# liuyuan-pal/Gen6D

Measured on NVIDIA H100. Metric: poses/sec end-to-end (128^2 crop, 64 refs, 3 refine iters), higher is better.
Workload: dtype f32

## Files before the change

### gen6d_b200/csrc/conv_tc.cu

```cuda
#include <cuda_fp16.h>
#include <string.h>

#include "tc_common.cuh"

namespace g6d {

constexpr int TC_BM = 128;
constexpr int TC_PRODUCER_WARPS = 8;
constexpr int TC_CONSUMER_WARPS = 8;
constexpr int TC_THREADS = (TC_PRODUCER_WARPS + TC_CONSUMER_WARPS) * 32;
constexpr int TC_ISSUER = TC_PRODUCER_WARPS * 32;
constexpr int TC_PRODUCER_REGS = 96, TC_CONSUMER_REGS = 160;
static_assert(TC_PRODUCER_WARPS * TC_PRODUCER_REGS + TC_CONSUMER_WARPS * TC_CONSUMER_REGS <= 65536 / 32, "register file of one SM");
constexpr int TC_FOLD_PRODUCER_REGS = 40, TC_FOLD_CONSUMER_REGS = 216;
static_assert(TC_PRODUCER_WARPS * TC_FOLD_PRODUCER_REGS + TC_CONSUMER_WARPS * TC_FOLD_CONSUMER_REGS <= 65536 / 32, "register file of one SM");
static_assert(TC_BM == 64 * (TC_CONSUMER_WARPS / 4), "one 64-row wgmma tile per consumer warpgroup");
constexpr int TC_MAX_K_PER_CHAIN = 2048;

template <int KIND> struct KindCfg;
template <> struct KindCfg<G6D_TC_TF32> {
    static constexpr int BK = 32;
    static constexpr int NV = 1;
    static constexpr float CROSS = 1.f;
};
template <> struct KindCfg<G6D_TC_F16> {
    static constexpr int BK = 64;
    static constexpr int NV = 2;
    static constexpr float CROSS = 1.f / 2048.f;
};
constexpr float F16_LO_SCALE = 2048.f;
constexpr int TC2_RING = 2, FLAT_RING = 3;
__host__ __device__ __forceinline__ int f16_k_source(int p) {
    const int c = p >> 3, i = p & 7;
    return i < 4 ? 4 * c + i : 32 + 4 * c + (i - 4);
}

struct ConvTcP {
    const float* x; const float* bias; const float* ps; const float* pb;
    float* y; float* ws;
    int B, D, H, W, Cin, ics, ico, Cout, kd, kh, kw, stride, pd, ph, pw, Do, Ho, Wo, ocs, oco, pro, act;
    long long group_rows;
    int M, K, kblocks, splits, kb_per_split;
    double* stats; long long stats_rows;
    int split_in;
    int reuse_order;
    int fold;
};

__device__ __forceinline__ void kblock_src(const ConvTcP& p, int sp, int it, int& tap, int& cb) {
    if (p.reuse_order) {
        const int taps2 = p.kh * p.kw;
        const int u = it / taps2, t = it - u * taps2;
        cb = sp * (p.kb_per_split / (taps2 * p.kd)) + u / p.kd;
        tap = (u % p.kd) * taps2 + t;
    } else {
        const int cblocks = p.Cin / 64, kb = sp * p.kb_per_split + it;
        tap = kb / cblocks;
        cb = kb - tap * cblocks;
    }
}

struct KbIter {
    int kx, ky, kz, cb;
    __device__ __forceinline__ void start(const ConvTcP& p, int sp, int it) {
        int tap;
        kblock_src(p, sp, it, tap, cb);
        kx = tap % p.kw;
        const int tq = tap / p.kw;
        ky = tq % p.kh;
        kz = tq / p.kh;
    }
    __device__ __forceinline__ void next(const ConvTcP& p) {
        if (p.reuse_order) {
            if (++kx < p.kw) return;
            kx = 0;
            if (++ky < p.kh) return;
            ky = 0;
            if (++kz < p.kd) return;
            kz = 0; ++cb;
// ... 167 lines not shown
    for (int i = 0; i < BN / 8; ++i) {
#pragma unroll
        for (int e = 0; e < 2; ++e) {
            const float y0 = dst0 ? cross[4 * i + e] : 0.f, y1 = dst1 ? cross[4 * i + 2 + e] : 0.f;
            const float2 s = slice_moments(y0, y1);
            const int n = n_base + 8 * i + cq + e;
            if (lane < 4 && n < Cout) {
                atomicAdd(stats + (group * Cout + n) * 2, (double)s.x);
                atomicAdd(stats + (group * Cout + n) * 2 + 1, (double)s.y);
            }
        }
    }
}

template <int BN, int KIND>
__device__ __forceinline__ void epilogue_tile(float (&acc)[AccCfg<BN>::NMAIN][BN / 2], float (&cross)[BN / 2], int n_acc,
                                              float* dst0, float* dst1, int n_base, int Cout, const float* __restrict__ bias,
                                              int act, bool partial, bool vec2, double* __restrict__ stats, long long group,
                                              int lane) {
    sum_chains<BN, KIND>(acc, cross, n_acc);
    store_tile<BN>(cross, dst0, dst1, n_base, Cout, bias, act, partial, vec2, stats, group, lane);
}

constexpr int TC2_PF_BYTES = 12 * 128;

template <int BN> struct Tc2Cfg {
    static constexpr int A_BYTES = TC_BM * 128;
    static constexpr int B_BYTES = BN * 128;
    static constexpr int STAGE_BYTES = 2 * A_BYTES + 2 * B_BYTES;
    static constexpr int STAGES = (208 * 1024) / STAGE_BYTES > 6 ? 6 : (208 * 1024) / STAGE_BYTES;
    static constexpr int SMEM_BYTES = STAGES * STAGE_BYTES + 1024 + 256;
};

struct Tc2Work { int m_tiles, n_tiles, total; };

template <int BN, int KIND, bool FOLD>
__global__ void __launch_bounds__(TC_THREADS, 1)
conv_tc2_kernel(const ConvTcP p, const Tc2Work wk, const __grid_constant__ CUtensorMap map_hi,
                const __grid_constant__ CUtensorMap map_lo, const __grid_constant__ CUtensorMap map_a) {
    using Cfg = Tc2Cfg<BN>;
    using KC = KindCfg<KIND>;
    constexpr int NPW = TC_PRODUCER_WARPS;
    constexpr int STAGES = Cfg::STAGES;
    constexpr int NMAIN = AccCfg<BN>::NMAIN;
    constexpr int BK = KC::BK, NV = KC::NV;
    constexpr int RSTEP = NPW * 4;
    constexpr int ROWS = TC_BM / RSTEP;
    constexpr int RING = TC2_RING;
    constexpr int PF = TC2_PF_BYTES / 128;
    extern __shared__ uint8_t smem_raw[];
    const uint32_t base = (smem_u32(smem_raw) + 1023u) & ~1023u;
    const uint32_t bar_base = base + STAGES * Cfg::STAGE_BYTES;
    auto a_hi = [&](int s) { return base + s * Cfg::STAGE_BYTES; };
    auto a_lo = [&](int s) { return base + s * Cfg::STAGE_BYTES + Cfg::A_BYTES; };
    auto b_hi = [&](int s) { return base + s * Cfg::STAGE_BYTES + 2 * Cfg::A_BYTES; };
    auto b_lo = [&](int s) { return base + s * Cfg::STAGE_BYTES + 2 * Cfg::A_BYTES + Cfg::B_BYTES; };
    auto full_a = [&](int s) { return bar_base + 8 * s; };
    auto full_b = [&](int s) { return bar_base + 8 * (STAGES + s); };
    auto empty = [&](int s) { return bar_base + 8 * (2 * STAGES + s); };

    const int warp = threadIdx.x >> 5, lane = threadIdx.x & 31;
    if (threadIdx.x == TC_ISSUER) {
        for (int s = 0; s < STAGES; ++s) {
            mbar_init(full_a(s), p.split_in ? 1 : NPW);
            mbar_init(full_b(s), 1);
            mbar_init(empty(s), TC_CONSUMER_WARPS);
        }
        fence_barrier_init();
        asm volatile("prefetch.tensormap [%0];" ::"l"(&map_hi) : "memory");
        asm volatile("prefetch.tensormap [%0];" ::"l"(&map_lo) : "memory");
        if (p.split_in) asm volatile("prefetch.tensormap [%0];" ::"l"(&map_a) : "memory");
    }
    __syncthreads();

    auto decode = [&](int w, int& mt, int& nt, int& sp) {
        nt = w % wk.n_tiles; w /= wk.n_tiles;
        mt = w % wk.m_tiles;
        sp = w / wk.m_tiles;
    };
    auto kblocks_of = [&](int sp) { return min(p.kblocks, sp * p.kb_per_split + p.kb_per_split) - sp * p.kb_per_split; };
    const int chains = FOLD ? p.splits : 1;
    auto chain_of = [&](int j, int& mt, int& nt, int& sp) {
        const int w = blockIdx.x + (j / chains) * gridDim.x;
        if (w >= wk.total) return false;
        decode(w, mt, nt, sp);
        sp += j % chains;
        return true;
    };

    if (warp < NPW) {
        setmaxnreg_dec<FOLD ? TC_FOLD_PRODUCER_REGS : TC_PRODUCER_REGS>();
        if (FOLD || p.split_in) {
            if (threadIdx.x == 0) {
                const bool vol = p.D > 1 || p.kd > 1;
                int g = 0;
                int mt, nt, sp;
                for (int j = 0; chain_of(j, mt, nt, sp); ++j) {
                    const int nkb = kblocks_of(sp);
                    int m = mt * TC_BM;
                    const int xo = m % p.Wo; m /= p.Wo;
                    const int yo = m % p.Ho; m /= p.Ho;
                    const int zo = m % p.Do;
                    const int b = m / p.Do;
                    KbIter pf, k;
                    pf.start(p, sp, 0);
                    k = pf;
                    auto prefetch = [&]() {
                        const int kc = pf.tap(p) * p.Cin + pf.cb * BK;
                        tma_prefetch_2d(&map_hi, kc, nt * BN);
                        tma_prefetch_2d(&map_lo, kc, nt * BN);
                        pf.next(p);
                    };
#pragma unroll 1
                    for (int i = 0; i < min(nkb, PF - 1); ++i) prefetch();
                    for (int it = 0; it < nkb; ++it, ++g, k.next(p)) {
                        if (it + PF - 1 < nkb) prefetch();
                        const int tap = k.tap(p), cb = k.cb;
                        const uint16_t ox = (uint16_t)k.kx, oy = (uint16_t)k.ky, oz = (uint16_t)k.kz;
                        const int s = g % STAGES;
                        mbar_wait(empty(s), ((g / STAGES) & 1) ^ 1, 1, g);
                        mbar_expect_tx(full_b(s), 2 * Cfg::B_BYTES);
                        tma_load_2d(b_hi(s), &map_hi, full_b(s), tap * p.Cin + cb * BK, nt * BN);
                        tma_load_2d(b_lo(s), &map_lo, full_b(s), tap * p.Cin + cb * BK, nt * BN);
                        mbar_expect_tx(full_a(s), 2 * Cfg::A_BYTES);
                        if (vol) {
                            tma_im2col_5d(a_hi(s), &map_a, full_a(s), 2 * BK * cb, xo - p.pw, yo - p.ph, zo - p.pd, b, ox, oy, oz);
// ... 75 lines not shown
                }
                if (e == 0) mbar_wait(empty(s), (n_use & 1) ^ 1, 1, g_it);
#pragma unroll
                for (int j = 0; j < ROWS; ++j) {
                    const int r = r0 + RSTEP * j;
                    const uint32_t so = r * 128 + ((chunk ^ (r & 7)) << 4);
                    split_store<KIND>(a_hi(s) + so, a_lo(s) + so, v[q][j], e);
                }
                if (e == NV - 1) {
                    fence_proxy_async();
                    __syncwarp();
                    if (lane == 0) mbar_arrive(full_a(s));
                }
            };
            const int ncol = nkb * NV;
#pragma unroll
            for (int q = 0; q < RING - 1; ++q)
                if (q < ncol) issue_loads(q, q % NV);
            for (int u = 0; u < ncol; u += RING) {
#pragma unroll
                for (int q = 0; q < RING; ++q) {
                    if (u + q < ncol) {
                        if (u + q + RING - 1 < ncol) issue_loads((q + RING - 1) % RING, (u + q + RING - 1) % NV);
                        process(q, (u + q) % NV, (u + q) / NV);
                    }
                }
            }
            git += nkb;
        }
    } else {
        setmaxnreg_inc<FOLD ? TC_FOLD_CONSUMER_REGS : TC_CONSUMER_REGS>();
        const int cw = warp - NPW;
        const uint32_t a_row = (cw >> 2) * 64 * 128;
        const bool issuer = !FOLD && threadIdx.x == TC_ISSUER && !p.split_in;
        int lw = blockIdx.x, lit = 0, lg = 0;
        auto load_next = [&]() {
            int mt, nt, sp, nkb = 0;
            for (; lw < wk.total; lw += gridDim.x, lit = 0) {
                decode(lw, mt, nt, sp);
                nkb = kblocks_of(sp);
                if (lit < nkb) break;
            }
            if (lw >= wk.total) return;
            const int kb_begin = sp * p.kb_per_split;
            if (lit == 0) {
                for (int i = 0; i < min(nkb, PF); ++i) {
                    tma_prefetch_2d(&map_hi, (kb_begin + i) * BK, nt * BN);
                    tma_prefetch_2d(&map_lo, (kb_begin + i) * BK, nt * BN);
                }
            } else if (lit + PF - 1 < nkb) {
                tma_prefetch_2d(&map_hi, (kb_begin + lit + PF - 1) * BK, nt * BN);
                tma_prefetch_2d(&map_lo, (kb_begin + lit + PF - 1) * BK, nt * BN);
            }
            const int s = lg % STAGES;
            mbar_wait(empty(s), ((lg / STAGES) & 1) ^ 1, 3, lg);
            mbar_expect_tx(full_b(s), 2 * Cfg::B_BYTES);
            tma_load_2d(b_hi(s), &map_hi, full_b(s), (kb_begin + lit) * BK, nt * BN);
            tma_load_2d(b_lo(s), &map_lo, full_b(s), (kb_begin + lit) * BK, nt * BN);
            ++lit; ++lg;
        };
        auto release = [&](int g) {
            __syncwarp();
            if (lane == 0) mbar_arrive(empty(g % STAGES));
            if (issuer) load_next();
        };
        if (issuer)
            for (int i = 0; i < STAGES; ++i) load_next();

        float acc[NMAIN][BN / 2];
        float cross[BN / 2];
        float run[FOLD ? BN / 2 : 1];
        int g = 0;
        int mt, nt, sp;
        for (int j = 0; chain_of(j, mt, nt, sp); ++j) {
            const int nkb = kblocks_of(sp);
            zero_acc<BN, NMAIN>(acc, cross);
            for (int it0 = 0; it0 < nkb; it0 += NMAIN) {
#pragma unroll
                for (int a = 0; a < NMAIN; ++a) {
                    const int it = it0 + a;
                    if (it < nkb) {
                        const int s = g % STAGES;
                        mbar_wait(full_a(s), (g / STAGES) & 1, 4, g);
                        mbar_wait(full_b(s), (g / STAGES) & 1, 5, g);
                        mma_stage<BN, KIND>(acc[a], cross, a_hi(s) + a_row, a_lo(s) + a_row, b_hi(s), b_lo(s));
                        wgmma_wait<1>();
                        if (it > 0) release(g - 1);
                        ++g;
                    }
                }
            }
            wgmma_wait<0>();
            if (nkb > 0) release(g - 1);

            sum_chains<BN, KIND>(acc, cross, nkb < NMAIN ? nkb : NMAIN);
            if constexpr (FOLD) {
#pragma unroll
                for (int jj = 0; jj < BN / 2; ++jj) run[jj] = (sp == 0 ? 0.f : run[jj]) + cross[jj];
                if (sp < p.splits - 1) continue;
#pragma unroll
                for (int jj = 0; jj < BN / 2; ++jj) cross[jj] = run[jj];
            }
            const bool partial = p.splits > 1 && !FOLD;
            const int n_base = nt * BN;
            const int m0 = mt * TC_BM + 16 * cw + (lane >> 2), m1 = m0 + 8;
            float* out = partial ? p.ws + (long long)sp * p.M * p.Cout + n_base : p.y + p.oco + n_base;
            const long long ld = partial ? p.Cout : p.ocs;
            const bool vec2 = partial ? (p.Cout & 1) == 0
                                      : ((p.ocs & 1) == 0 && (p.oco & 1) == 0 && (reinterpret_cast<uintptr_t>(p.y) & 7) == 0);
            store_tile<BN>(cross, m0 < p.M ? out + m0 * ld : nullptr, m1 < p.M ? out + m1 * ld : nullptr, n_base, p.Cout, p.bias,
                           p.act, partial, vec2, p.stats, (long long)(mt * TC_BM + 16 * cw) / p.stats_rows, lane);
        }
    }
}


__global__ void conv_tc_reduce_kernel(const float* __restrict__ ws, const float* __restrict__ bias,
                                      float* __restrict__ y, int M, int Cout, int splits, int ocs, int oco, int act) {
    const long long i = (long long)blockIdx.x * blockDim.x + threadIdx.x;
    if (i >= (long long)M * Cout) return;
    const int n = (int)(i % Cout);
    const long long m = i / Cout;
    float v = 0.f;
    for (int s = 0; s < splits; ++s) v += ws[(long long)s * M * Cout + i];
    if (bias) v += bias[n];
    y[m * ocs + oco + n] = tc_act(v, act);
}

template <int SPLITS>
__device__ __forceinline__ float4 sum_splits4(const float4* __restrict__ ws4, long long slab4, long long i4, int splits) {
    float4 p[SPLITS > 0 ? SPLITS : 1];
    float4 v = make_float4(0.f, 0.f, 0.f, 0.f);
    if constexpr (SPLITS > 0) {
#pragma unroll
        for (int s = 0; s < SPLITS; ++s) p[s] = __ldg(ws4 + s * slab4 + i4);
#pragma unroll
        for (int s = 0; s < SPLITS; ++s) { v.x += p[s].x; v.y += p[s].y; v.z += p[s].z; v.w += p[s].w; }
    } else {
        for (int s = 0; s < splits; ++s) {
            const float4 q = __ldg(ws4 + s * slab4 + i4);
            v.x += q.x; v.y += q.y; v.z += q.z; v.w += q.w;
        }
    }
// ... 113 lines not shown
    if (!enc) { set_error("g6d_conv_tc: cuTensorMapEncodeTiled unavailable"); return G6D_ECUDA; }
    cuuint64_t dims[2] = {(cuuint64_t)K, (cuuint64_t)rows};
    cuuint64_t strides[1] = {(cuuint64_t)K * kind_esize(kind)};
    cuuint32_t box[2] = {(cuuint32_t)kind_bk(kind), (cuuint32_t)bn};
    cuuint32_t estr[2] = {1, 1};
    CUresult r = enc(map, kind == G6D_TC_F16 ? CU_TENSOR_MAP_DATA_TYPE_FLOAT16 : CU_TENSOR_MAP_DATA_TYPE_FLOAT32, 2,
                     const_cast<void*>(w), dims, strides, box, estr,
                     CU_TENSOR_MAP_INTERLEAVE_NONE, CU_TENSOR_MAP_SWIZZLE_128B, CU_TENSOR_MAP_L2_PROMOTION_L2_256B,
                     CU_TENSOR_MAP_FLOAT_OOB_FILL_NONE);
    if (r != CUDA_SUCCESS) { set_error("g6d_conv_tc: cuTensorMapEncodeTiled failed (%d)", (int)r); return G6D_ECUDA; }
    return G6D_OK;
}

typedef CUresult (*EncodeIm2colFn)(CUtensorMap*, CUtensorMapDataType, cuuint32_t, void*, const cuuint64_t*, const cuuint64_t*,
                                   const int*, const int*, cuuint32_t, cuuint32_t, const cuuint32_t*, CUtensorMapInterleave,
                                   CUtensorMapSwizzle, CUtensorMapL2promotion, CUtensorMapFloatOOBfill);

static EncodeIm2colFn get_encode_im2col_fn() {
    static EncodeIm2colFn fn = nullptr;
    static bool tried = false;
    if (!tried) {
        tried = true;
        void* sym = nullptr;
        cudaDriverEntryPointQueryResult qres;
        if (cudaGetDriverEntryPoint("cuTensorMapEncodeIm2col", &sym, cudaEnableDefault, &qres) == cudaSuccess &&
            qres == cudaDriverEntryPointSuccess)
            fn = reinterpret_cast<EncodeIm2colFn>(sym);
    }
    return fn;
}

static bool split_input_rank5(const g6d_conv_desc* d) { return d->D > 1 || d->kd > 1; }

static int make_split_input_map(CUtensorMap* map, const void* xs, const g6d_conv_desc* d) {
    EncodeIm2colFn enc = get_encode_im2col_fn();
    if (!enc) { set_error("g6d_conv_tc: cuTensorMapEncodeIm2col unavailable"); return G6D_ECUDA; }
    const cuuint64_t C2 = 2ull * d->Cin;
    const cuuint32_t rank = split_input_rank5(d) ? 5 : 4;
    cuuint64_t dims[5] = {C2, (cuuint64_t)d->W, (cuuint64_t)d->H, (cuuint64_t)d->D, (cuuint64_t)d->B};
    cuuint64_t strides[4] = {C2 * 2, C2 * 2 * d->W, C2 * 2 * d->W * d->H, C2 * 2 * d->W * d->H * d->D};
    if (rank == 4) dims[3] = d->B;
    int lower[3] = {-d->pw, -d->ph, -d->pd};
    int upper[3] = {d->pw - (d->kw - 1), d->ph - (d->kh - 1), d->pd - (d->kd - 1)};
    cuuint32_t estr[5] = {1, 1, 1, 1, 1};
    CUresult r = enc(map, CU_TENSOR_MAP_DATA_TYPE_FLOAT16, rank, const_cast<void*>(xs), dims, strides, lower, upper, 64, TC_BM, estr,
                     CU_TENSOR_MAP_INTERLEAVE_NONE, CU_TENSOR_MAP_SWIZZLE_128B, CU_TENSOR_MAP_L2_PROMOTION_L2_256B,
                     CU_TENSOR_MAP_FLOAT_OOB_FILL_NONE);
    if (r != CUDA_SUCCESS) { set_error("g6d_conv_tc: cuTensorMapEncodeIm2col failed (%d)", (int)r); return G6D_ECUDA; }
    return G6D_OK;
}

static int tc_block_n(int Cout) { return Cout > 64 ? 128 : (Cout > 32 ? 64 : 32); }
static int tc_nmain(int bn) { return bn == 32 ? AccCfg<32>::NMAIN : (bn == 64 ? AccCfg<64>::NMAIN : AccCfg<128>::NMAIN); }

static bool tc2_dims_ok(const g6d_conv_desc* d) {
    return d->D + d->pd + 8 < 256 && d->H + d->ph + 8 < 4096 && d->W + d->pw + 8 < 4096 &&
           (long long)d->D * d->H * d->W < (1ll << 30) && d->group_rows < (1ll << 31);
}

static int fill_tc_params(const g6d_conv_desc* d, int kind, ConvTcP& p) {
    G6D_REQUIRE(d != nullptr, "g6d_conv_tc: null desc");
    G6D_REQUIRE(kind == G6D_TC_TF32 || kind == G6D_TC_F16, "g6d_conv_tc: bad operand kind %d", kind);
    G6D_REQUIRE(d->B > 0 && d->D > 0 && d->H > 0 && d->W > 0 && d->Cin > 0, "g6d_conv_tc: bad dims");
    G6D_REQUIRE(d->Cout >= 16, "g6d_conv_tc: Cout (%d) must be at least 16", d->Cout);
    G6D_REQUIRE(d->kd > 0 && d->kh > 0 && d->kw > 0 && d->stride > 0, "g6d_conv_tc: bad kernel/stride");
    const int bk = kind_bk(kind);
    G6D_REQUIRE((d->Cin % bk) == 0, "g6d_conv_tc: Cin (%d) must be a multiple of %d", d->Cin, bk);
    G6D_REQUIRE((d->in_cstride & 3) == 0 && (d->in_coff & 3) == 0, "g6d_conv_tc: in_cstride/in_coff must be multiples of 4");
    G6D_REQUIRE(d->in_coff + d->Cin <= d->in_cstride, "g6d_conv_tc: input channel slice out of row");
    G6D_REQUIRE(d->out_coff + d->Cout <= d->out_cstride, "g6d_conv_tc: output channel slice out of row");
    G6D_REQUIRE(tc2_dims_ok(d), "g6d_conv_tc: spatial extent too large for the tensor-core kernel");
    const int Do = (d->D + 2 * d->pd - d->kd) / d->stride + 1;
    const int Ho = (d->H + 2 * d->ph - d->kh) / d->stride + 1;
    const int Wo = (d->W + 2 * d->pw - d->kw) / d->stride + 1;
    G6D_REQUIRE(Do > 0 && Ho > 0 && Wo > 0 && Do == d->Do && Ho == d->Ho && Wo == d->Wo, "g6d_conv_tc: output dims mismatch");
    G6D_REQUIRE(d->prologue >= 0 && d->prologue <= 3 && d->act >= 0 && d->act <= 2, "g6d_conv_tc: bad prologue/act");
    const long long M = (long long)d->B * Do * Ho * Wo;
    const long long K = (long long)d->kd * d->kh * d->kw * d->Cin;
    G6D_REQUIRE(M < (1ll << 31) && K < (1ll << 31), "g6d_conv_tc: problem too large");
    p.B = d->B; p.D = d->D; p.H = d->H; p.W = d->W; p.Cin = d->Cin; p.ics = d->in_cstride; p.ico = d->in_coff;
    p.Cout = d->Cout; p.kd = d->kd; p.kh = d->kh; p.kw = d->kw; p.stride = d->stride; p.pd = d->pd; p.ph = d->ph;
    p.pw = d->pw; p.Do = Do; p.Ho = Ho; p.Wo = Wo; p.ocs = d->out_cstride; p.oco = d->out_coff; p.pro = d->prologue;
    p.act = d->act; p.group_rows = d->group_rows > 0 ? d->group_rows : 1;
    p.M = (int)M; p.K = (int)K; p.kblocks = (int)(K / bk);
    const int bn = tc_block_n(d->Cout);
    const long long ctas = (long long)ceil_div(M, TC_BM) * ceil_div(d->Cout, bn);
    const int min_kb = 256 / bk;
    int splits = 1;
    if (ctas < kNumSMs && p.kblocks >= 2 * min_kb) {
        splits = (int)(kNumSMs / ctas);
        splits = splits > p.kblocks / min_kb ? p.kblocks / min_kb : splits;
        splits = splits < 1 ? 1 : splits;
    }
    const int nmain = tc_nmain(bn);
    const int chain = d->max_chain_k > 0 ? d->max_chain_k * nmain : (K > TC_MAX_K_PER_CHAIN ? TC_MAX_K_PER_CHAIN * nmain : 0);
    const int max_kb = chain > bk ? chain / bk : 1;
    const int min_splits = chain > 0 ? (p.kblocks + max_kb - 1) / max_kb : 1;
    splits = splits < min_splits ? min_splits : splits;
    splits = splits > 64 ? 64 : splits;
    p.kb_per_split = (p.kblocks + splits - 1) / splits;
    p.splits = (p.kblocks + p.kb_per_split - 1) / p.kb_per_split;
    return G6D_OK;
}

template <int BN, int KIND, bool FOLD>
static int launch_tc2(const ConvTcP& p, const CUtensorMap& mh, const CUtensorMap& ml, const CUtensorMap& ma, cudaStream_t st) {
    using Cfg = Tc2Cfg<BN>;
    static bool configured = false;
    if (!configured) {
        cudaError_t e = cudaFuncSetAttribute(conv_tc2_kernel<BN, KIND, FOLD>, cudaFuncAttributeMaxDynamicSharedMemorySize, Cfg::SMEM_BYTES);
        if (e != cudaSuccess) { set_error("g6d_conv_tc: cannot opt in to %d B of shared memory: %s", Cfg::SMEM_BYTES, cudaGetErrorString(e)); return G6D_ECUDA; }
        configured = true;
    }
    Tc2Work wk;
    wk.m_tiles = ceil_div(p.M, TC_BM); wk.n_tiles = ceil_div(p.Cout, BN);
    const long long total = (long long)wk.m_tiles * wk.n_tiles * (FOLD ? 1 : p.splits);
    wk.total = (int)total;
    const int grid = total < kNumSMs ? (int)total : kNumSMs;
    conv_tc2_kernel<BN, KIND, FOLD><<<grid, TC_THREADS, Cfg::SMEM_BYTES, st>>>(p, wk, mh, ml, ma);
    G6D_CHECK_LAUNCH("g6d_conv_tc");
    return G6D_OK;
}

__global__ void split_tf32_kernel(const float* __restrict__ in, float* __restrict__ hi, float* __restrict__ lo, long long n) {
    const long long i = (long long)blockIdx.x * blockDim.x + threadIdx.x;
    if (i >= n) return;
    const float v = in[i];
    const float h = to_tf32(v);
    hi[i] = h;
    lo[i] = to_tf32(v - h);
}
__device__ __forceinline__ void split_f16_scalar(float v, __half& h, __half& l) {
    uint32_t hh, ll;
    split_f16x2(v, 0.f, hh, ll);
    h = __ushort_as_half((unsigned short)(hh & 0xffffu));
    l = __ushort_as_half((unsigned short)(ll & 0xffffu));
}
__global__ void split_f16_kernel(const float* __restrict__ in, __half* __restrict__ hi, __half* __restrict__ lo, long long n) {
    const long long i = (long long)blockIdx.x * blockDim.x + threadIdx.x;
    if (i >= n) return;
    split_f16_scalar(in[(i & ~63ll) + f16_k_source((int)(i & 63))], hi[i], lo[i]);
}

__global__ void split_input_f16_kernel(const float* __restrict__ x, int ics, int ico, int Cin, long long rows,
                                       long long plane, int pro, const float* __restrict__ ps, const float* __restrict__ pb,
                                       long long group_rows, __half* __restrict__ out) {
    const long long i = (long long)blockIdx.x * blockDim.x + threadIdx.x;
    const int chunks = Cin / 8;
    if (i >= rows * chunks) return;
    const long long r = i / chunks;
    const int q = (int)(i - r * chunks), cb = q >> 3, c = q & 7;
    const float* src = x + r * ics + ico + cb * 64 + 4 * c;
// ... 343 lines not shown
    }
    dim3 grid((unsigned)((long long)p.B * p.Do * p.tiles_per_plane), ceil_div(p.Cout, BN), p.splits);
    conv_tcflat_kernel<BN, KIND><<<grid, TC_THREADS, smem, st>>>(p, mh, ml);
    G6D_CHECK_LAUNCH("g6d_conv_tc(flat)");
    return G6D_OK;
}

struct ConvPlan {
    ConvTcP tc;
    ConvFlatP flat;
    bool use_flat;
    int bn, splits, flat_smem;
    long long split_in_off;
    long long ws_bytes;
};

constexpr double TC_FOLD_SLACK = 0.15;

static bool fold_ok(const ConvPlan& pl) {
    if (pl.use_flat || !pl.tc.split_in || pl.splits < 2) return false;
    const long long T = (long long)ceil_div(pl.tc.M, TC_BM) * ceil_div(pl.tc.Cout, pl.bn), S = pl.splits;
    return (double)(ceil_div(T, kNumSMs) * S) <= (1.0 + TC_FOLD_SLACK) * (double)ceil_div(T * S, kNumSMs);
}

static bool split_input_ok(const g6d_conv_desc* d, int kind, int flags, bool use_flat) {
    if (use_flat || kind != G6D_TC_F16 || (d->prologue != G6D_PRO_NONE && !(flags & G6D_TC_PRENORM)) || d->stride != 1 ||
        d->kd * d->kh * d->kw == 1)
        return false;
    if (!split_input_rank5(d)) return d->kw <= 64 && d->kh <= 64 && d->pw < 64 && d->ph < 64;
    auto corners_ok = [](int k, int pad) { return k <= 16 && pad <= 16 && pad - (k - 1) >= -16 && pad - (k - 1) <= 15; };
    return (flags & G6D_TC_REUSE_IM2COL) && corners_ok(d->kw, d->pw) && corners_ok(d->kh, d->ph) && corners_ok(d->kd, d->pd);
}

static int make_plan(const g6d_conv_desc* d, int kind, int flags, ConvPlan& pl) {
    G6D_REQUIRE((flags & ~(G6D_TC_PRENORM | G6D_TC_REUSE_IM2COL | G6D_TC_FOLD_SPLITS)) == 0, "g6d_conv_tc: bad flags %d", flags);
    const int rc = fill_tc_params(d, kind, pl.tc);
    if (rc != G6D_OK) return rc;
    pl.use_flat = fill_flat_params(d, kind, pl.flat, &pl.flat_smem);
    pl.tc.reuse_order = 0;
    if (pl.use_flat && (flags & G6D_TC_REUSE_IM2COL) && split_input_ok(d, kind, flags, false)) {
        pl.use_flat = false;
        pl.tc.reuse_order = 1;
        pl.tc.kb_per_split = pl.flat.cb_per_split * d->kd * d->kh * d->kw;
        pl.tc.splits = pl.flat.splits;
    }
    pl.bn = tc_block_n(d->Cout);
    pl.splits = pl.use_flat ? pl.flat.splits : pl.tc.splits;
    pl.tc.split_in = split_input_ok(d, kind, flags, pl.use_flat) ? 1 : 0;
    pl.tc.fold = (flags & G6D_TC_FOLD_SPLITS) && fold_ok(pl) ? 1 : 0;
    const long long partials =
        pl.splits > 1 && !pl.tc.fold ? (long long)pl.splits * pl.tc.M * pl.tc.Cout * (long long)sizeof(float) : 0;
    pl.split_in_off = (partials + 255) / 256 * 256;
    pl.ws_bytes = pl.tc.split_in
                      ? pl.split_in_off + (long long)d->B * d->D * d->H * d->W * d->Cin * 2 * (long long)sizeof(__half)
                      : partials;
    return G6D_OK;
}

static bool stats_ok(const ConvPlan& pl, long long stats_rows) {
    if (stats_rows <= 0 || stats_rows % 32 != 0 || pl.tc.M % stats_rows != 0) return false;
    return !(pl.use_flat || pl.tc.reuse_order) || stats_rows % ((long long)pl.flat.Ho * pl.flat.Wo) == 0;
}

template <class P>
static void bind_tensors(P& p, const float* x, const float* bias, const float* ps, const float* pb, float* y, void* ws,
                         double* stats, long long stats_rows) {
    p.x = x; p.bias = bias; p.ps = ps; p.pb = pb; p.y = y; p.ws = static_cast<float*>(ws);
    p.stats = stats; p.stats_rows = stats ? stats_rows : 1;
}

template <int BN, int KIND>
static int launch_plan(const ConvPlan& pl, const CUtensorMap& mh, const CUtensorMap& ml, const CUtensorMap& ma, cudaStream_t st) {
    if (pl.use_flat) return launch_flat<BN, KIND>(pl.flat, pl.flat_smem, mh, ml, st);
    if constexpr (KIND == G6D_TC_F16)
        if (pl.tc.fold) return launch_tc2<BN, KIND, true>(pl.tc, mh, ml, ma, st);
    return launch_tc2<BN, KIND, false>(pl.tc, mh, ml, ma, st);
}
template <int KIND>
static int dispatch(const ConvPlan& pl, const CUtensorMap& mh, const CUtensorMap& ml, const CUtensorMap& ma, cudaStream_t st) {
    if (pl.bn == 128) return launch_plan<128, KIND>(pl, mh, ml, ma, st);
    if (pl.bn == 64) return launch_plan<64, KIND>(pl, mh, ml, ma, st);
    return launch_plan<32, KIND>(pl, mh, ml, ma, st);
}

}

using namespace g6d;

extern "C" int g6d_conv_tc_debug(int* host_out8) {
    G6D_REQUIRE(host_out8 != nullptr, "g6d_conv_tc_debug: null");
    cudaError_t e = cudaDeviceSynchronize();
    if (e != cudaSuccess) { set_error("g6d_conv_tc_debug: sync: %s", cudaGetErrorString(e)); return G6D_ECUDA; }
    e = cudaMemcpyFromSymbol(host_out8, g_tc_timeout, sizeof(int) * 8);
    if (e != cudaSuccess) { set_error("g6d_conv_tc_debug: %s", cudaGetErrorString(e)); return G6D_ECUDA; }
    int zeros[8] = {0, 0, 0, 0, 0, 0, 0, 0};
    cudaMemcpyToSymbol(g_tc_timeout, zeros, sizeof(zeros));
    return G6D_OK;
}

extern "C" int g6d_conv_tc_supported(const g6d_conv_desc* d, int kind) {
    ConvPlan pl{};
    return make_plan(d, kind, 0, pl) == G6D_OK ? 1 : 0;
}

extern "C" long long g6d_conv_tc_workspace_bytes_ex(const g6d_conv_desc* desc, int kind, int flags) {
    ConvPlan pl{};
    if (make_plan(desc, kind, flags, pl) != G6D_OK) return -1;
    return pl.ws_bytes;
}

extern "C" long long g6d_conv_tc_workspace_bytes(const g6d_conv_desc* desc, int kind) {
    return g6d_conv_tc_workspace_bytes_ex(desc, kind, 0);
}

extern "C" int g6d_conv_tc_stats_supported(const g6d_conv_desc* desc, int kind, long long stats_rows) {
    ConvPlan pl{};
    return make_plan(desc, kind, 0, pl) == G6D_OK && stats_ok(pl, stats_rows) ? 1 : 0;
}

extern "C" int g6d_conv_tc_plan_ex(const g6d_conv_desc* desc, int kind, int flags, int* out4) {
    G6D_REQUIRE(out4 != nullptr, "g6d_conv_tc_plan: null output");
    ConvPlan pl{};
    const int rc = make_plan(desc, kind, flags, pl);
    if (rc != G6D_OK) return rc;
    out4[0] = pl.use_flat ? 1 : 0;
    out4[1] = pl.bn;
    out4[2] = pl.splits;
    out4[3] = pl.tc.split_in;
    return G6D_OK;
}

extern "C" int g6d_conv_tc_plan_v2(const g6d_conv_desc* desc, int kind, int flags, int* out, int n) {
    G6D_REQUIRE(out != nullptr && n > 0, "g6d_conv_tc_plan_v2: null output");
    ConvPlan pl{};
    const int rc = make_plan(desc, kind, flags, pl);
    if (rc != G6D_OK) return rc;
    const int v[5] = {pl.use_flat ? 1 : 0, pl.bn, pl.splits, pl.tc.split_in, pl.tc.fold};
    for (int i = 0; i < n && i < 5; ++i) out[i] = v[i];
    return G6D_OK;
}

extern "C" int g6d_conv_tc_plan(const g6d_conv_desc* desc, int kind, int* out4) {
    return g6d_conv_tc_plan_ex(desc, kind, 0, out4);
}

extern "C" int g6d_conv_tc_ex(const g6d_conv_desc* desc, const float* x, const void* w_hi, const void* w_lo, int w_rows,
                              int kind, const float* bias, const float* pro_scale, const float* pro_shift, float* y,
                              void* ws, double* stats, long long stats_rows, int flags, g6d_stream_t stream) {
    ConvPlan pl{};
    int rc = make_plan(desc, kind, flags, pl);
    if (rc != G6D_OK) return rc;
    const ConvTcP& p = pl.tc;
    if (stats) G6D_REQUIRE(stats_ok(pl, stats_rows), "g6d_conv_tc: fused statistics need groups of whole 32-row slices / planes (stats_rows %lld)", stats_rows);
    G6D_REQUIRE(x && w_hi && w_lo && y, "g6d_conv_tc: null tensor pointer");
    G6D_REQUIRE(w_rows >= p.Cout, "g6d_conv_tc: weight rows (%d) < Cout (%d)", w_rows, p.Cout);
    if (p.pro != G6D_PRO_NONE) G6D_REQUIRE(pro_scale && pro_shift, "g6d_conv_tc: prologue operands missing");
    if (pl.ws_bytes > 0) G6D_REQUIRE(ws != nullptr, "g6d_conv_tc: workspace required (%lld bytes)", pl.ws_bytes);
    cudaStream_t st = as_stream(stream);
    if (stats) {
        cudaError_t e = cudaMemsetAsync(stats, 0, sizeof(double) * 2 * (p.M / stats_rows) * p.Cout, st);
        if (e != cudaSuccess) { set_error("g6d_conv_tc: memset: %s", cudaGetErrorString(e)); return G6D_ECUDA; }
    }
    const bool flat_moments = stats && p.reuse_order && pl.splits == 1;
    const bool fold_moments = stats && p.fold;
    if (pl.use_flat) bind_tensors(pl.flat, x, bias, pro_scale, pro_shift, y, ws, stats, stats_rows);
    else bind_tensors(pl.tc, x, bias, pro_scale, pro_shift, y, ws, flat_moments || fold_moments ? nullptr : stats, stats_rows);
    CUtensorMap mh, ml, ma;
    if ((rc = make_weight_map(&mh, w_hi, w_rows, p.K, pl.bn, kind)) != G6D_OK) return rc;
    if ((rc = make_weight_map(&ml, w_lo, w_rows, p.K, pl.bn, kind)) != G6D_OK) return rc;
    memset(&ma, 0, sizeof(ma));
    if (p.split_in) {
        __half* xs = reinterpret_cast<__half*>(static_cast<char*>(ws) + pl.split_in_off);
        if ((rc = make_split_input_map(&ma, xs, desc)) != G6D_OK) return rc;
        const long long plane = (long long)p.D * p.H * p.W, rows = p.B * plane, n = rows * (p.Cin / 8);
        split_input_f16_kernel<<<ceil_div(n, 256), 256, 0, st>>>(x, p.ics, p.ico, p.Cin, rows, plane, p.pro, pro_scale,
                                                                  pro_shift, p.group_rows, xs);
        G6D_CHECK_LAUNCH("g6d_conv_tc(split input)");
    }
    rc = kind == G6D_TC_F16 ? dispatch<G6D_TC_F16>(pl, mh, ml, ma, st) : dispatch<G6D_TC_TF32>(pl, mh, ml, ma, st);
    if (rc != G6D_OK) return rc;
    if (flat_moments) {
        const ConvFlatP& f = pl.flat;
        dim3 grid((unsigned)((long long)f.B * f.Do), ceil_div(f.Cout, 8));
        flat_moments_kernel<<<grid, 256, 0, st>>>(y, f.ocs, f.oco, f.Cout, f.Ho, f.Wo, f.Wp, f.tiles_per_plane * TC_CONSUMER_WARPS,
                                                  stats, stats_rows);
        G6D_CHECK_LAUNCH("g6d_conv_tc(moments)");
    }
    if (fold_moments) {
        fold_moments_kernel<<<dim3(ceil_div(p.M, 32), ceil_div(p.Cout, 64)), 256, 0, st>>>(y, p.M, p.Cout, p.ocs, p.oco, stats,
                                                                                          stats_rows);
        G6D_CHECK_LAUNCH("g6d_conv_tc(fold moments)");
    }
    if (pl.splits > 1 && !p.fold) {
        launch_reduce(static_cast<float*>(ws), bias, y, p.M, p.Cout, pl.splits, p.ocs, p.oco, p.act, stats, stats_rows, st);
        G6D_CHECK_LAUNCH("g6d_conv_tc(split reduce)");
    }
    return G6D_OK;
}

extern "C" int g6d_conv_tc(const g6d_conv_desc* desc, const float* x, const void* w_hi, const void* w_lo, int w_rows,
                           int kind, const float* bias, const float* pro_scale, const float* pro_shift, float* y,
                           void* ws, double* stats, long long stats_rows, g6d_stream_t stream) {
    return g6d_conv_tc_ex(desc, x, w_hi, w_lo, w_rows, kind, bias, pro_scale, pro_shift, y, ws, stats, stats_rows, 0, stream);
}

extern "C" int g6d_split_operand(const float* in, void* hi, void* lo, long long n, int kind, g6d_stream_t stream) {
// ... 73 lines not shown
```

### gen6d_b200/ops.py

```python
import ctypes as C
import os
from dataclasses import dataclass
from typing import Optional

import torch

from . import _lib
from ._lib import ACT_LEAKY01, ACT_NONE, ACT_RELU, PRO_AFFINE, PRO_AFFINE_RELU, PRO_CORR, PRO_NONE


WARP_JOB_BYTES = 88


def _stream():
    return C.c_void_p(torch.cuda.current_stream().cuda_stream)


def _p(t, dtype=torch.float32):
    if t is None:
        return None
    if not (t.is_cuda and t.dtype == dtype and t.is_contiguous()):
        raise ValueError(f'expected a contiguous CUDA {dtype} tensor, got {t.dtype} {t.device} '
                         f'contiguous={t.is_contiguous()} shape={tuple(t.shape)}')
    return C.c_void_p(t.data_ptr())
# ... 482 lines not shown

def conv(x, pc, prologue=PRO_NONE, pro_scale=None, pro_shift=None, group_rows=1, act=ACT_NONE,
         in_coff=0, out=None, out_coff=0, stats_rows=None, prenorm=False, reuse_im2col=False, fold_splits=False):
    four = x.dim() == 4
    if four:
        B, H, W, cs = x.shape
        D = 1
    else:
        B, D, H, W, cs = x.shape
    kd, kh, kw = pc.k
    pd, ph, pw = pc.pad
    s = pc.stride
    Do, Ho, Wo = (D + 2 * pd - kd) // s + 1, (H + 2 * ph - kh) // s + 1, (W + 2 * pw - kw) // s + 1
    if out is None:
        shape = (B, Ho, Wo, pc.cout) if four else (B, Do, Ho, Wo, pc.cout)
        out = torch.empty(shape, device=x.device, dtype=torch.float32)
    d = _lib.ConvDesc(B=B, D=D, H=H, W=W, Cin=pc.cin, in_cstride=cs, in_coff=in_coff, Cout=pc.cout, kd=kd, kh=kh,
                      kw=kw, stride=s, pd=pd, ph=ph, pw=pw, Do=Do, Ho=Ho, Wo=Wo, out_cstride=out.shape[-1],
                      out_coff=out_coff, prologue=prologue, group_rows=group_rows, act=act, max_chain_k=pc.max_chain_k)
    work = 2.0 * B * Do * Ho * Wo * pc.cout * kd * kh * kw * pc.cin
    M = B * Do * Ho * Wo
    stats = None
    if pc.w_hi is not None and conv_path() == 'tc' and _lib.lib().g6d_conv_tc_supported(C.byref(d), pc.kind):
        flags = ((_lib.TC_PRENORM if prenorm else 0) | (_lib.TC_REUSE_IM2COL if reuse_im2col else 0)
                 | (_lib.TC_FOLD_SPLITS if fold_splits else 0))
        nbytes = _lib.lib().g6d_conv_tc_workspace_bytes_ex(C.byref(d), pc.kind, flags)
        if nbytes < 0:
            _lib.check(-1, 'g6d_conv_tc_workspace_bytes_ex')
        ws = torch.empty(nbytes // 4, device=x.device, dtype=torch.float32) if nbytes > 0 else None
        fuse = stats_rows is not None and _lib.lib().g6d_conv_tc_stats_supported(C.byref(d), pc.kind, stats_rows)
        if fuse:
            stats = torch.empty(M // stats_rows, pc.cout, 2, device=x.device, dtype=torch.float64)
        def tag(d=d, kind=pc.kind, flags=flags):
            plan = (C.c_int * 5)()
            _lib.check(_lib.lib().g6d_conv_tc_plan_v2(C.byref(d), kind, flags, plan, 5), 'g6d_conv_tc_plan_v2')
            a_op = (' prenorm' if prologue != PRO_NONE else ' im2col') if plan[3] else ''
            if flags & _lib.TC_REUSE_IM2COL and plan[3]:
                plain = (C.c_int * 4)()
                _lib.check(_lib.lib().g6d_conv_tc_plan_ex(C.byref(d), kind, flags & ~_lib.TC_REUSE_IM2COL, plain),
                           'g6d_conv_tc_plan_ex')
                a_op += '-ro' if plain[0] else ''
            return (f'M={M} N={pc.cout} K={kd * kh * kw * pc.cin} k={kd}x{kh}x{kw} s={s} pro={prologue} '
                    f'{"reuse" if plan[0] else "persist"} BN={plan[1]} splits={plan[2]}{" fold" if plan[4] else ""}{a_op}')
        _call('g6d_conv_tc_ex', C.byref(d), _p(x), _p(pc.w_hi, pc.w_hi.dtype), _p(pc.w_lo, pc.w_lo.dtype), pc.w_hi.shape[0],
              pc.kind, _p(pc.bias), _p(pro_scale), _p(pro_shift), _p(out), _p(ws), _p(stats, torch.float64), stats_rows or 0,
              flags, _stream(), work=work, tag=tag, key='g6d_conv_tc')
    else:
        if pc.w is None:
            raise _lib.Gen6DLibraryError('this operand was packed for the tensor-core path only and the problem is not supported there')
        nbytes = _lib.lib().g6d_conv_workspace_bytes(C.byref(d))
        if nbytes < 0:
            _lib.check(-1, 'g6d_conv_workspace_bytes')
        ws = torch.empty(nbytes // 4, device=x.device, dtype=torch.float32) if nbytes > 0 else None
        _call('g6d_conv', C.byref(d), _p(x), _p(pc.w), _p(pc.bias), _p(pro_scale), _p(pro_shift), _p(out), _p(ws), _stream(),
              work=work)
    if stats_rows is None:
        return out
    if stats is None:
        stats = instnorm_partial(out, rows_per_group=stats_rows, channels=pc.cout, coff=out_coff)
    return out, stats


def vgg_first_block(x, pc):
    B, H, W, _ = x.shape
    out = torch.empty(B, H // 2, W // 2, 64, device=x.device, dtype=torch.float32)
    _call('g6d_vgg_first_block', _p(x), _p(pc.w), _p(pc.bias), _p(out), B, H, W, _stream())
    return out


def linear_smallm(x, w, bias, act=ACT_NONE):
    M, K = x.shape
    N = w.shape[0]
    out = torch.empty(M, N, device=x.device, dtype=torch.float32)
    _call('g6d_linear_smallm', _p(x), _p(w), _p(bias), _p(out), M, N, K, act, _stream())
# ... 145 lines not shown
```

Before: 122.7.

## Reuse one im2col input box across kw taps in split-input TC conv

Adds an x-reuse (XR) variant of the warp-specialized conv kernel. For each (ky,kz,cb) it loads a single wider im2col box of TC_BM+kw-1 rows, and consumers reach each kx tap by offsetting rows inside that box, so the A operand is not reloaded once per horizontal tap. Output rows are indexed in a padded-width space (Wp = Wo+kw-1), and the epilogue skips the padding columns, which wastes some MMA work on rows that are thrown away. The path is limited to f16 split-input, reuse-order plans with BN=64, and it adds separate box and weight rings with their own barriers.

Result: faster. 126.7 (median of 6 runs) (+3.3%).

```diff
diff --git a/gen6d_b200/csrc/conv_tc.cu b/gen6d_b200/csrc/conv_tc.cu
--- a/gen6d_b200/csrc/conv_tc.cu
+++ b/gen6d_b200/csrc/conv_tc.cu
@@ -45,6 +45,7 @@
     int split_in;
     int reuse_order;
     int fold;
+    int xr, Wp, Mp, xr_rows;
 };
 
 __device__ __forceinline__ void kblock_src(const ConvTcP& p, int sp, int it, int& tap, int& cb) {
@@ -278,13 +279,24 @@
     static constexpr int SMEM_BYTES = STAGES * STAGE_BYTES + 1024 + 256;
 };
 
+template <int BN> struct Tc2XrCfg {
+    static constexpr int BOX_ROWS = 144;
+    static constexpr int BOX_BYTES = BOX_ROWS * 128;
+    static constexpr int BOXES = 3;
+    static constexpr int B_BYTES = BN * 128;
+    static constexpr int B_STAGES = 6;
+    static constexpr int SMEM_BYTES = BOXES * 2 * BOX_BYTES + B_STAGES * 2 * B_BYTES + 1024 + 256;
+};
+static_assert(Tc2XrCfg<64>::SMEM_BYTES <= 227 * 1024, "x-reuse rings of BN 64");
+
 struct Tc2Work { int m_tiles, n_tiles, total; };
 
-template <int BN, int KIND, bool FOLD>
+template <int BN, int KIND, bool FOLD, bool XR>
 __global__ void __launch_bounds__(TC_THREADS, 1)
 conv_tc2_kernel(const ConvTcP p, const Tc2Work wk, const __grid_constant__ CUtensorMap map_hi,
                 const __grid_constant__ CUtensorMap map_lo, const __grid_constant__ CUtensorMap map_a) {
     using Cfg = Tc2Cfg<BN>;
+    using XC = Tc2XrCfg<BN>;
     using KC = KindCfg<KIND>;
     constexpr int NPW = TC_PRODUCER_WARPS;
     constexpr int STAGES = Cfg::STAGES;
@@ -304,9 +316,32 @@
     auto full_a = [&](int s) { return bar_base + 8 * s; };
     auto full_b = [&](int s) { return bar_base + 8 * (STAGES + s); };
     auto empty = [&](int s) { return bar_base + 8 * (2 * STAGES + s); };
+    auto box_hi = [&](int s) { return base + s * 2 * XC::BOX_BYTES; };
+    auto box_lo = [&](int s) { return base + s * 2 * XC::BOX_BYTES + XC::BOX_BYTES; };
+    const uint32_t xb_base = base + XC::BOXES * 2 * XC::BOX_BYTES;
+    auto xb_hi = [&](int s) { return xb_base + s * 2 * XC::B_BYTES; };
+    auto xb_lo = [&](int s) { return xb_base + s * 2 * XC::B_BYTES + XC::B_BYTES; };
+    const uint32_t xbar = xb_base + XC::B_STAGES * 2 * XC::B_BYTES;
+    auto box_full = [&](int s) { return xbar + 8 * s; };
+    auto box_empty = [&](int s) { return xbar + 8 * (XC::BOXES + s); };
+    auto xb_full = [&](int s) { return xbar + 8 * (2 * XC::BOXES + s); };
+    auto xb_empty = [&](int s) { return xbar + 8 * (2 * XC::BOXES + XC::B_STAGES + s); };
 
     const int warp = threadIdx.x >> 5, lane = threadIdx.x & 31;
-    if (threadIdx.x == TC_ISSUER) {
+    if (XR && threadIdx.x == TC_ISSUER) {
+        for (int s = 0; s < XC::BOXES; ++s) {
+            mbar_init(box_full(s), 1);
+            mbar_init(box_empty(s), TC_CONSUMER_WARPS);
+        }
+        for (int s = 0; s < XC::B_STAGES; ++s) {
+            mbar_init(xb_full(s), 1);
+            mbar_init(xb_empty(s), TC_CONSUMER_WARPS);
+        }
+        fence_barrier_init();
+        asm volatile("prefetch.tensormap [%0];" ::"l"(&map_hi) : "memory");
+        asm volatile("prefetch.tensormap [%0];" ::"l"(&map_lo) : "memory");
+        asm volatile("prefetch.tensormap [%0];" ::"l"(&map_a) : "memory");
+    } else if (threadIdx.x == TC_ISSUER) {
         for (int s = 0; s < STAGES; ++s) {
             mbar_init(full_a(s), p.split_in ? 1 : NPW);
             mbar_init(full_b(s), 1);
@@ -336,8 +371,56 @@
 
     if (warp < NPW) {
         setmaxnreg_dec<FOLD ? TC_FOLD_PRODUCER_REGS : TC_PRODUCER_REGS>();
-        if (FOLD || p.split_in) {
-            if (threadIdx.x == 0) {
+        if (XR && threadIdx.x == 0) {
+            const bool vol = p.D > 1 || p.kd > 1;
+            const uint32_t box_tx = 2u * p.xr_rows * 128u;
+            int g = 0, gb = 0;
+            int mt, nt, sp;
+            for (int j = 0; chain_of(j, mt, nt, sp); ++j) {
+                const int nkb = kblocks_of(sp);
+                int m = mt * TC_BM;
+                const int xo = m % p.Wp; m /= p.Wp;
+                const int yo = m % p.Ho; m /= p.Ho;
+                const int zo = m % p.Do;
+                const int b = m / p.Do;
+                KbIter pf, k;
+                pf.start(p, sp, 0);
+                k = pf;
+                auto prefetch = [&]() {
+                    const int kc = pf.tap(p) * p.Cin + pf.cb * BK;
+                    tma_prefetch_2d(&map_hi, kc, nt * BN);
+                    tma_prefetch_2d(&map_lo, kc, nt * BN);
+                    pf.next(p);
+                };
+#pragma unroll 1
+                for (int i = 0; i < min(nkb, PF - 1); ++i) prefetch();
+                for (int it = 0; it < nkb; ++it, ++g, k.next(p)) {
+                    if (it + PF - 1 < nkb) prefetch();
+                    if (k.kx == 0) {
+                        const int s = gb % XC::BOXES;
+                        const uint16_t oy = (uint16_t)k.ky, oz = (uint16_t)k.kz;
+                        mbar_wait(box_empty(s), ((gb / XC::BOXES) & 1) ^ 1, 6, gb);
+                        mbar_expect_tx(box_full(s), box_tx);
+                        if (vol) {
+                            tma_im2col_5d(box_hi(s), &map_a, box_full(s), 2 * BK * k.cb, xo - p.pw, yo - p.ph, zo - p.pd, b, 0, oy, oz);
+                            tma_im2col_5d(box_lo(s), &map_a, box_full(s), 2 * BK * k.cb + BK, xo - p.pw, yo - p.ph, zo - p.pd, b, 0, oy, oz);
+                        } else {
+                            tma_im2col_4d(box_hi(s), &map_a, box_full(s), 2 * BK * k.cb, xo - p.pw, yo - p.ph, b, 0, oy);
+                            tma_im2col_4d(box_lo(s), &map_a, box_full(s), 2 * BK * k.cb + BK, xo - p.pw, yo - p.ph, b, 0, oy);
+                        }
+                        ++gb;
+                    }
+                    const int s = g % XC::B_STAGES;
+                    mbar_wait(xb_empty(s), ((g / XC::B_STAGES) & 1) ^ 1, 1, g);
+                    mbar_expect_tx(xb_full(s), 2 * XC::B_BYTES);
+                    tma_load_2d(xb_hi(s), &map_hi, xb_full(s), k.tap(p) * p.Cin + k.cb * BK, nt * BN);
+                    tma_load_2d(xb_lo(s), &map_lo, xb_full(s), k.tap(p) * p.Cin + k.cb * BK, nt * BN);
+                }
+            }
+            return;
+        }
+        if (XR || FOLD || p.split_in) {
+            if (!XR && threadIdx.x == 0) {
                 const bool vol = p.D > 1 || p.kd > 1;
                 int g = 0;
                 int mt, nt, sp;
@@ -479,7 +562,7 @@
         setmaxnreg_inc<FOLD ? TC_FOLD_CONSUMER_REGS : TC_CONSUMER_REGS>();
         const int cw = warp - NPW;
         const uint32_t a_row = (cw >> 2) * 64 * 128;
-        const bool issuer = !FOLD && threadIdx.x == TC_ISSUER && !p.split_in;
+        const bool issuer = !FOLD && !XR && threadIdx.x == TC_ISSUER && !p.split_in;
         int lw = blockIdx.x, lit = 0, lg = 0;
         auto load_next = [&]() {
             int mt, nt, sp, nkb = 0;
@@ -518,10 +601,46 @@
         float cross[BN / 2];
         float run[FOLD ? BN / 2 : 1];
         int g = 0;
+        int gb = 0, rb = 0;
+        auto xr_release = [&](int g, bool box_done) {
+            __syncwarp();
+            if (lane == 0) {
+                mbar_arrive(xb_empty(g % XC::B_STAGES));
+                if (box_done) mbar_arrive(box_empty(rb % XC::BOXES));
+            }
+            if (box_done) ++rb;
+        };
         int mt, nt, sp;
         for (int j = 0; chain_of(j, mt, nt, sp); ++j) {
             const int nkb = kblocks_of(sp);
             zero_acc<BN, NMAIN>(acc, cross);
+            if constexpr (XR) {
+                int kx = 0;
+                bool box_done = false;
+                for (int it0 = 0; it0 < nkb; it0 += NMAIN) {
+#pragma unroll
+                    for (int a = 0; a < NMAIN; ++a) {
+                        const int it = it0 + a;
+                        if (it < nkb) {
+                            if (kx == 0) {
+                                mbar_wait(box_full(gb % XC::BOXES), (gb / XC::BOXES) & 1, 7, gb);
+                                ++gb;
+                            }
+                            const int s = g % XC::B_STAGES, sb = (gb - 1) % XC::BOXES;
+                            mbar_wait(xb_full(s), (g / XC::B_STAGES) & 1, 5, g);
+                            const uint32_t sh = a_row + kx * 128;
+                            mma_stage<BN, KIND>(acc[a], cross, box_hi(sb) + sh, box_lo(sb) + sh, xb_hi(s), xb_lo(s));
+                            wgmma_wait<1>();
+                            if (it > 0) xr_release(g - 1, box_done);
+                            box_done = kx == p.kw - 1;
+                            ++g;
+                            if (++kx == p.kw) kx = 0;
+                        }
+                    }
+                }
+                wgmma_wait<0>();
+                if (nkb > 0) xr_release(g - 1, true);
+            } else {
             for (int it0 = 0; it0 < nkb; it0 += NMAIN) {
 #pragma unroll
                 for (int a = 0; a < NMAIN; ++a) {
@@ -539,6 +658,7 @@
             }
             wgmma_wait<0>();
             if (nkb > 0) release(g - 1);
+            }
 
             sum_chains<BN, KIND>(acc, cross, nkb < NMAIN ? nkb : NMAIN);
             if constexpr (FOLD) {
@@ -555,7 +675,16 @@
             const long long ld = partial ? p.Cout : p.ocs;
             const bool vec2 = partial ? (p.Cout & 1) == 0
                                       : ((p.ocs & 1) == 0 && (p.oco & 1) == 0 && (reinterpret_cast<uintptr_t>(p.y) & 7) == 0);
-            store_tile<BN>(cross, m0 < p.M ? out + m0 * ld : nullptr, m1 < p.M ? out + m1 * ld : nullptr, n_base, p.Cout, p.bias,
+            auto dst = [&](int m) -> float* {
+                if constexpr (XR) {
+                    if (m >= p.Mp) return nullptr;
+                    const int q = m / p.Wp, xp = m - q * p.Wp;
+                    return xp < p.Wo ? out + ((long long)q * p.Wo + xp) * ld : nullptr;
+                } else {
+                    return m < p.M ? out + m * ld : nullptr;
+                }
+            };
+            store_tile<BN>(cross, dst(m0), dst(m1), n_base, p.Cout, p.bias,
                            p.act, partial, vec2, p.stats, (long long)(mt * TC_BM + 16 * cw) / p.stats_rows, lane);
         }
     }
@@ -735,7 +864,7 @@
 
 static bool split_input_rank5(const g6d_conv_desc* d) { return d->D > 1 || d->kd > 1; }
 
-static int make_split_input_map(CUtensorMap* map, const void* xs, const g6d_conv_desc* d) {
+static int make_split_input_map(CUtensorMap* map, const void* xs, const g6d_conv_desc* d, int xr_rows) {
     EncodeIm2colFn enc = get_encode_im2col_fn();
     if (!enc) { set_error("g6d_conv_tc: cuTensorMapEncodeIm2col unavailable"); return G6D_ECUDA; }
     const cuuint64_t C2 = 2ull * d->Cin;
@@ -744,9 +873,10 @@
     cuuint64_t strides[4] = {C2 * 2, C2 * 2 * d->W, C2 * 2 * d->W * d->H, C2 * 2 * d->W * d->H * d->D};
     if (rank == 4) dims[3] = d->B;
     int lower[3] = {-d->pw, -d->ph, -d->pd};
-    int upper[3] = {d->pw - (d->kw - 1), d->ph - (d->kh - 1), d->pd - (d->kd - 1)};
+    int upper[3] = {d->pw - (xr_rows ? 0 : d->kw - 1), d->ph - (d->kh - 1), d->pd - (d->kd - 1)};
     cuuint32_t estr[5] = {1, 1, 1, 1, 1};
-    CUresult r = enc(map, CU_TENSOR_MAP_DATA_TYPE_FLOAT16, rank, const_cast<void*>(xs), dims, strides, lower, upper, 64, TC_BM, estr,
+    CUresult r = enc(map, CU_TENSOR_MAP_DATA_TYPE_FLOAT16, rank, const_cast<void*>(xs), dims, strides, lower, upper, 64,
+                     xr_rows ? xr_rows : TC_BM, estr,
                      CU_TENSOR_MAP_INTERLEAVE_NONE, CU_TENSOR_MAP_SWIZZLE_128B, CU_TENSOR_MAP_L2_PROMOTION_L2_256B,
                      CU_TENSOR_MAP_FLOAT_OOB_FILL_NONE);
     if (r != CUDA_SUCCESS) { set_error("g6d_conv_tc: cuTensorMapEncodeIm2col failed (%d)", (int)r); return G6D_ECUDA; }
@@ -806,21 +936,21 @@
     return G6D_OK;
 }
 
-template <int BN, int KIND, bool FOLD>
+template <int BN, int KIND, bool FOLD, bool XR>
 static int launch_tc2(const ConvTcP& p, const CUtensorMap& mh, const CUtensorMap& ml, const CUtensorMap& ma, cudaStream_t st) {
-    using Cfg = Tc2Cfg<BN>;
+    constexpr int SMEM = XR ? Tc2XrCfg<BN>::SMEM_BYTES : Tc2Cfg<BN>::SMEM_BYTES;
     static bool configured = false;
     if (!configured) {
-        cudaError_t e = cudaFuncSetAttribute(conv_tc2_kernel<BN, KIND, FOLD>, cudaFuncAttributeMaxDynamicSharedMemorySize, Cfg::SMEM_BYTES);
-        if (e != cudaSuccess) { set_error("g6d_conv_tc: cannot opt in to %d B of shared memory: %s", Cfg::SMEM_BYTES, cudaGetErrorString(e)); return G6D_ECUDA; }
+        cudaError_t e = cudaFuncSetAttribute(conv_tc2_kernel<BN, KIND, FOLD, XR>, cudaFuncAttributeMaxDynamicSharedMemorySize, SMEM);
+        if (e != cudaSuccess) { set_error("g6d_conv_tc: cannot opt in to %d B of shared memory: %s", SMEM, cudaGetErrorString(e)); return G6D_ECUDA; }
         configured = true;
     }
     Tc2Work wk;
-    wk.m_tiles = ceil_div(p.M, TC_BM); wk.n_tiles = ceil_div(p.Cout, BN);
+    wk.m_tiles = ceil_div(XR ? p.Mp : p.M, TC_BM); wk.n_tiles = ceil_div(p.Cout, BN);
     const long long total = (long long)wk.m_tiles * wk.n_tiles * (FOLD ? 1 : p.splits);
     wk.total = (int)total;
     const int grid = total < kNumSMs ? (int)total : kNumSMs;
-    conv_tc2_kernel<BN, KIND, FOLD><<<grid, TC_THREADS, Cfg::SMEM_BYTES, st>>>(p, wk, mh, ml, ma);
+    conv_tc2_kernel<BN, KIND, FOLD, XR><<<grid, TC_THREADS, SMEM, st>>>(p, wk, mh, ml, ma);
     G6D_CHECK_LAUNCH("g6d_conv_tc");
     return G6D_OK;
 }
@@ -1230,6 +1360,12 @@
     return (flags & G6D_TC_REUSE_IM2COL) && corners_ok(d->kw, d->pw) && corners_ok(d->kh, d->ph) && corners_ok(d->kd, d->pd);
 }
 
+static bool xr_ok(const g6d_conv_desc* d, const ConvPlan& pl) {
+    if (!pl.tc.split_in || !pl.tc.reuse_order || pl.bn != 64 || d->kw < 2 || d->kw > 17) return false;
+    if (split_input_rank5(d) && d->pw > 15) return false;
+    return (long long)pl.tc.M / pl.tc.Wo * (pl.tc.Wo + d->kw - 1) < (1ll << 31);
+}
+
 static int make_plan(const g6d_conv_desc* d, int kind, int flags, ConvPlan& pl) {
     G6D_REQUIRE((flags & ~(G6D_TC_PRENORM | G6D_TC_REUSE_IM2COL | G6D_TC_FOLD_SPLITS)) == 0, "g6d_conv_tc: bad flags %d", flags);
     const int rc = fill_tc_params(d, kind, pl.tc);
@@ -1246,6 +1382,12 @@
     pl.splits = pl.use_flat ? pl.flat.splits : pl.tc.splits;
     pl.tc.split_in = split_input_ok(d, kind, flags, pl.use_flat) ? 1 : 0;
     pl.tc.fold = (flags & G6D_TC_FOLD_SPLITS) && fold_ok(pl) ? 1 : 0;
+    pl.tc.xr = xr_ok(d, pl) ? 1 : 0;
+    if (pl.tc.xr) {
+        pl.tc.Wp = pl.tc.Wo + d->kw - 1;
+        pl.tc.Mp = (int)((long long)pl.tc.M / pl.tc.Wo * pl.tc.Wp);
+        pl.tc.xr_rows = (TC_BM + d->kw - 1 + 7) / 8 * 8;
+    }
     const long long partials =
         pl.splits > 1 && !pl.tc.fold ? (long long)pl.splits * pl.tc.M * pl.tc.Cout * (long long)sizeof(float) : 0;
     pl.split_in_off = (partials + 255) / 256 * 256;
@@ -1270,9 +1412,13 @@
 template <int BN, int KIND>
 static int launch_plan(const ConvPlan& pl, const CUtensorMap& mh, const CUtensorMap& ml, const CUtensorMap& ma, cudaStream_t st) {
     if (pl.use_flat) return launch_flat<BN, KIND>(pl.flat, pl.flat_smem, mh, ml, st);
-    if constexpr (KIND == G6D_TC_F16)
-        if (pl.tc.fold) return launch_tc2<BN, KIND, true>(pl.tc, mh, ml, ma, st);
-    return launch_tc2<BN, KIND, false>(pl.tc, mh, ml, ma, st);
+    if constexpr (KIND == G6D_TC_F16) {
+        if constexpr (BN == 64)
+            if (pl.tc.xr) return pl.tc.fold ? launch_tc2<BN, KIND, true, true>(pl.tc, mh, ml, ma, st)
+                                            : launch_tc2<BN, KIND, false, true>(pl.tc, mh, ml, ma, st);
+        if (pl.tc.fold) return launch_tc2<BN, KIND, true, false>(pl.tc, mh, ml, ma, st);
+    }
+    return launch_tc2<BN, KIND, false, false>(pl.tc, mh, ml, ma, st);
 }
 template <int KIND>
 static int dispatch(const ConvPlan& pl, const CUtensorMap& mh, const CUtensorMap& ml, const CUtensorMap& ma, cudaStream_t st) {
@@ -1333,8 +1479,8 @@
     ConvPlan pl{};
     const int rc = make_plan(desc, kind, flags, pl);
     if (rc != G6D_OK) return rc;
-    const int v[5] = {pl.use_flat ? 1 : 0, pl.bn, pl.splits, pl.tc.split_in, pl.tc.fold};
-    for (int i = 0; i < n && i < 5; ++i) out[i] = v[i];
+    const int v[6] = {pl.use_flat ? 1 : 0, pl.bn, pl.splits, pl.tc.split_in, pl.tc.fold, pl.tc.xr};
+    for (int i = 0; i < n && i < 6; ++i) out[i] = v[i];
     return G6D_OK;
 }
 
@@ -1369,7 +1515,7 @@
     memset(&ma, 0, sizeof(ma));
     if (p.split_in) {
         __half* xs = reinterpret_cast<__half*>(static_cast<char*>(ws) + pl.split_in_off);
-        if ((rc = make_split_input_map(&ma, xs, desc)) != G6D_OK) return rc;
+        if ((rc = make_split_input_map(&ma, xs, desc, p.xr ? p.xr_rows : 0)) != G6D_OK) return rc;
         const long long plane = (long long)p.D * p.H * p.W, rows = p.B * plane, n = rows * (p.Cin / 8);
         split_input_f16_kernel<<<ceil_div(n, 256), 256, 0, st>>>(x, p.ics, p.ico, p.Cin, rows, plane, p.pro, pro_scale,
                                                                   pro_shift, p.group_rows, xs);
diff --git a/gen6d_b200/ops.py b/gen6d_b200/ops.py
--- a/gen6d_b200/ops.py
+++ b/gen6d_b200/ops.py
@@ -538,14 +538,15 @@
         if fuse:
             stats = torch.empty(M // stats_rows, pc.cout, 2, device=x.device, dtype=torch.float64)
         def tag(d=d, kind=pc.kind, flags=flags):
-            plan = (C.c_int * 5)()
-            _lib.check(_lib.lib().g6d_conv_tc_plan_v2(C.byref(d), kind, flags, plan, 5), 'g6d_conv_tc_plan_v2')
+            plan = (C.c_int * 6)()
+            _lib.check(_lib.lib().g6d_conv_tc_plan_v2(C.byref(d), kind, flags, plan, 6), 'g6d_conv_tc_plan_v2')
             a_op = (' prenorm' if prologue != PRO_NONE else ' im2col') if plan[3] else ''
             if flags & _lib.TC_REUSE_IM2COL and plan[3]:
                 plain = (C.c_int * 4)()
                 _lib.check(_lib.lib().g6d_conv_tc_plan_ex(C.byref(d), kind, flags & ~_lib.TC_REUSE_IM2COL, plain),
                            'g6d_conv_tc_plan_ex')
                 a_op += '-ro' if plain[0] else ''
+            a_op += '-xr' if plan[5] else ''
             return (f'M={M} N={pc.cout} K={kd * kh * kw * pc.cin} k={kd}x{kh}x{kw} s={s} pro={prologue} '
                     f'{"reuse" if plan[0] else "persist"} BN={plan[1]} splits={plan[2]}{" fold" if plan[4] else ""}{a_op}')
         _call('g6d_conv_tc_ex', C.byref(d), _p(x), _p(pc.w_hi, pc.w_hi.dtype), _p(pc.w_lo, pc.w_lo.dtype), pc.w_hi.shape[0],
```
